# ZrrSkywalker/MonoDETR

Measured on NVIDIA H100. Metric: images/sec (1280x384, fwd+bwd), higher is better.
Workload: dtype f32 (BF16x3: error-compensated bf16 tensor-core products, fp32 accumulate)

## Files before the change

monodetr_b200/csrc/msda.cu:

```cuda
#include <cuda_runtime.h>
#include <stdint.h>

#include "../../include/monodetr_b200.h"
#include "launch.cuh"

namespace {

using namespace mdb;

constexpr int kMaxLevels = 8;
constexpr int kThreads = 256;

struct LevelInfo {
    int H[kMaxLevels];
    int W[kMaxLevels];
    int start[kMaxLevels];
};

__device__ __forceinline__ float4 ldg4(const float* p) { return __ldg(reinterpret_cast<const float4*>(p)); }

__device__ __forceinline__ void red_add_v4(float* addr, float a, float b, float c, float d) {
    asm volatile("red.global.add.v4.f32 [%0], {%1, %2, %3, %4};" ::"l"(addr), "f"(a), "f"(b), "f"(c), "f"(d)
                 : "memory");
}

__device__ __forceinline__ float fma_t(float a, float b, float c) { return fmaf(a, b, c); }
__device__ __forceinline__ double fma_t(double a, double b, double c) { return fma(a, b, c); }
__device__ __forceinline__ float floor_t(float a) { return floorf(a); }
__device__ __forceinline__ double floor_t(double a) { return floor(a); }

template <int LPU>
__global__ void __launch_bounds__(kThreads)
msda_fwd_vec_kernel(const float* __restrict__ value, const int64_t* __restrict__ shapes,
                    const int64_t* __restrict__ lsi, const float* __restrict__ loc,
                    const float* __restrict__ attn, int S, int M, int L, int Lq, long long n_units,
                    long long units_per_block, float* __restrict__ out) {
    constexpr int D = 4 * LPU;
    constexpr int UPW = 32 / LPU;
    constexpr int P = 4;
    __shared__ LevelInfo lv;
    if (threadIdx.x < L) {
        lv.H[threadIdx.x] = (int)shapes[2 * threadIdx.x];
        lv.W[threadIdx.x] = (int)shapes[2 * threadIdx.x + 1];
        lv.start[threadIdx.x] = (int)lsi[threadIdx.x];
    }
    __syncthreads();

    const int lane = threadIdx.x & 31;
    const int sub = lane / LPU;
    const int cl = lane % LPU;
    const int wib = threadIdx.x >> 5;
    const int pix = M * D;
    const long long u_begin = (long long)blockIdx.x * units_per_block;
    const long long u_end = min(n_units, u_begin + units_per_block);
// ... 134 lines not shown
#pragma unroll 1
        for (int half = 0; half < 2; ++half) {
            float2 xy = __ldg(reinterpret_cast<const float2*>(loc + (size_t)u * (L * P * 2)) + half * 8 + cl);
            float a;
            if constexpr (FUSED) {
                a = half ? e1 : e0;
                const int l = half ? lB : lA;
                const float* r = ref + ((size_t)(u / M) * L + l) * ref_dim;
                if (ref_dim == 2) {
                    xy.x = __ldg(r) + xy.x / (float)(half ? WB : WA);
                    xy.y = __ldg(r + 1) + xy.y / (float)(half ? HB : HA);
                } else {
                    xy.x = fmaf(xy.x, (__ldg(r + 2) + __ldg(r + 3)) * 0.5f / (float)P, __ldg(r));
                    xy.y = fmaf(xy.y, (__ldg(r + 4) + __ldg(r + 5)) * 0.5f / (float)P, __ldg(r + 1));
                }
            } else {
                a = __ldg(attn + (size_t)u * (L * P) + half * 8 + cl);
            }
            const PointSetup Sx = half ? setup_point(xy.x, xy.y, a, HB, WB, sB, pix) : setup_point(xy.x, xy.y, a, HA, WA, sA, pix);
#pragma unroll
            for (int jg = 0; jg < 4; ++jg) {
                float4 v[2][4];
                float w[2][4];
#pragma unroll
                for (int jj = 0; jj < 2; ++jj) {
                    const int j = jg * 2 + jj;
                    const int o00 = __shfl_sync(0xffffffffu, Sx.o00, j, 8);
                    const int dxo = __shfl_sync(0xffffffffu, Sx.dxo, j, 8);
                    const int dyo = __shfl_sync(0xffffffffu, Sx.dyo, j, 8);
#pragma unroll
                    for (int k = 0; k < 4; ++k) w[jj][k] = __shfl_sync(0xffffffffu, Sx.w[k], j, 8);
                    const float* p00 = vb + o00;
                    v[jj][0] = ldg4(p00);
                    v[jj][1] = ldg4(p00 + dxo);
                    v[jj][2] = ldg4(p00 + dyo);
                    v[jj][3] = ldg4(p00 + dyo + dxo);
                }
#pragma unroll
                for (int jj = 0; jj < 2; ++jj) {
#pragma unroll
                    for (int k = 0; k < 4; ++k) {
                        acc.x = fmaf(w[jj][k], v[jj][k].x, acc.x);
                        acc.y = fmaf(w[jj][k], v[jj][k].y, acc.y);
                        acc.z = fmaf(w[jj][k], v[jj][k].z, acc.z);
                        acc.w = fmaf(w[jj][k], v[jj][k].w, acc.w);
                    }
                }
            }
        }
        if (live) *reinterpret_cast<float4*>(out + (size_t)unit * D + cl * 4) = acc;
    }
}

template <int LPU, int L, bool FUSED = false, bool REFGRAD = false>
__global__ void __launch_bounds__(kThreads, 2)
msda_bwd_vec_kernel(const float* __restrict__ value, const int64_t* __restrict__ shapes,
                    const int64_t* __restrict__ lsi, const float* __restrict__ loc,
                    const float* __restrict__ attn, const float* __restrict__ grad_out, int S, int M,
                    int Lq, long long n_units, long long units_per_block, float* __restrict__ grad_value,
                    float* __restrict__ grad_loc, float* __restrict__ grad_attn, const float* __restrict__ ref = nullptr,
                    int ref_dim = 0, float* __restrict__ ref_part = nullptr) {
    static_assert(!FUSED || (LPU == 8 && L == 4), "fused pre-processing: D = 32, L = 4");
    static_assert(!REFGRAD || FUSED, "box partials: fused path only");
    constexpr int D = 4 * LPU;
    constexpr int UPW = 32 / LPU;
    constexpr int P = 4;
    constexpr int NLOC = 2 * L * P;
    constexpr int NV = 3 * L * P;
    constexpr int PER = NV / LPU;
    static_assert(NV % LPU == 0 && NLOC % LPU == 0, "butterfly needs divisibility");
    __shared__ LevelInfo lv;
    if (threadIdx.x < L) {
        lv.H[threadIdx.x] = (int)shapes[2 * threadIdx.x];
        lv.W[threadIdx.x] = (int)shapes[2 * threadIdx.x + 1];
        lv.start[threadIdx.x] = (int)lsi[threadIdx.x];
    }
    __syncthreads();

    const int lane = threadIdx.x & 31;
    const int sub = lane / LPU;
    const int cl = lane % LPU;
    const int wib = threadIdx.x >> 5;
    const int pix = M * D;
    const long long u_begin = (long long)blockIdx.x * units_per_block;
    const long long u_end = min(((n_units + UPW - 1) / UPW) * UPW, u_begin + units_per_block);

    for (long long unit = u_begin + wib * UPW + sub; unit < u_end; unit += (kThreads / 32) * UPW) {
        const bool live = unit < n_units;
        const long long u = live ? unit : 0;
        const int m = (int)(u % M);
        const long long b = u / ((long long)Lq * M);
        const size_t vbase = ((size_t)b * S * M + m) * D + cl * 4;
        const float* lp = loc + (size_t)u * L * P * 2;
        const float* ap = attn + (size_t)u * L * P;
        float4 g = ldg4(grad_out + (size_t)u * D + cl * 4);
        if (!live) g = make_float4(0.f, 0.f, 0.f, 0.f);
        [[maybe_unused]] float pa[2] = {0.f, 0.f}, px[2] = {0.f, 0.f}, py[2] = {0.f, 0.f};
        [[maybe_unused]] float sc[L][2];
        if constexpr (FUSED) {
            const float l0 = __ldg(ap + cl), l1 = __ldg(ap + 8 + cl);
            float mx = fmaxf(l0, l1);
            mx = fmaxf(mx, __shfl_xor_sync(0xffffffffu, mx, 4, 8));
            mx = fmaxf(mx, __shfl_xor_sync(0xffffffffu, mx, 2, 8));
            mx = fmaxf(mx, __shfl_xor_sync(0xffffffffu, mx, 1, 8));
            pa[0] = expf(l0 - mx); pa[1] = expf(l1 - mx);
            float sum = pa[0] + pa[1];
            sum += __shfl_xor_sync(0xffffffffu, sum, 4, 8);
            sum += __shfl_xor_sync(0xffffffffu, sum, 2, 8);
            sum += __shfl_xor_sync(0xffffffffu, sum, 1, 8);
            const float inv = 1.f / sum;
            pa[0] *= inv; pa[1] *= inv;
#pragma unroll
            for (int hf = 0; hf < 2; ++hf) {
                const int l = 2 * hf + (cl >> 2);
                const float2 o = __ldg(reinterpret_cast<const float2*>(lp) + hf * 8 + cl);
                const float* r = ref + ((size_t)(u / M) * L + l) * ref_dim;
                if (ref_dim == 2) {
                    px[hf] = __ldg(r) + o.x / (float)lv.W[l];
                    py[hf] = __ldg(r + 1) + o.y / (float)lv.H[l];
                } else {
                    px[hf] = fmaf(o.x, (__ldg(r + 2) + __ldg(r + 3)) * 0.5f / (float)P, __ldg(r));
                    py[hf] = fmaf(o.y, (__ldg(r + 4) + __ldg(r + 5)) * 0.5f / (float)P, __ldg(r + 1));
                }
            }
        }

        float vals[NV];
#pragma unroll
        for (int l = 0; l < L; ++l) {
            const int H = lv.H[l], W = lv.W[l];
            const size_t lbase = vbase + (size_t)lv.start[l] * pix;
            const float4 xy01 = ldg4(lp + l * 8);
            const float4 xy23 = ldg4(lp + l * 8 + 4);
            const float4 a4 = ldg4(ap + l * 4);
            float xs[4] = {xy01.x, xy01.z, xy23.x, xy23.z};
            float ys[4] = {xy01.y, xy01.w, xy23.y, xy23.w};
            float as[4] = {a4.x, a4.y, a4.z, a4.w};
            if constexpr (FUSED) {
                if (ref_dim == 2) {
                    sc[l][0] = 1.f / (float)W; sc[l][1] = 1.f / (float)H;
                } else {
                    const float* r = ref + ((size_t)(u / M) * L + l) * ref_dim;
                    sc[l][0] = (__ldg(r + 2) + __ldg(r + 3)) * 0.5f / (float)P;
                    sc[l][1] = (__ldg(r + 4) + __ldg(r + 5)) * 0.5f / (float)P;
                }
#pragma unroll
                for (int p = 0; p < P; ++p) {
                    xs[p] = __shfl_sync(0xffffffffu, px[l >> 1], 4 * (l & 1) + p, 8);
                    ys[p] = __shfl_sync(0xffffffffu, py[l >> 1], 4 * (l & 1) + p, 8);
                    as[p] = __shfl_sync(0xffffffffu, pa[l >> 1], 4 * (l & 1) + p, 8);
                }
            }
#pragma unroll
            for (int p = 0; p < P; ++p) {
                const float x = fmaf(xs[p], (float)W, -0.5f);
                const float y = fmaf(ys[p], (float)H, -0.5f);
                const bool inside = live && (y > -1.f) && (x > -1.f) && (y < (float)H) && (x < (float)W);
                const float xf = floorf(x), yf = floorf(y);
                const int x0 = (int)xf, y0 = (int)yf;
                const float lx = x - xf, ly = y - yf, hx = 1.f - lx, hy = 1.f - ly;
                const bool top = inside && (y0 >= 0), bot = inside && (y0 + 1 <= H - 1);
                const bool lef = (x0 >= 0), rig = (x0 + 1 <= W - 1);
                const long long o00 = (long long)lbase + ((long long)y0 * W + x0) * pix;
                const long long o01 = o00 + pix, o10 = o00 + (long long)W * pix, o11 = o10 + pix;
                const float4 z = make_float4(0.f, 0.f, 0.f, 0.f);
                const float4 v1 = (top && lef) ? ldg4(value + o00) : z;
                const float4 v2 = (top && rig) ? ldg4(value + o01) : z;
                const float4 v3 = (bot && lef) ? ldg4(value + o10) : z;
                const float4 v4 = (bot && rig) ? ldg4(value + o11) : z;
                const float a = as[p];
                const float w1 = hy * hx, w2 = hy * lx, w3 = ly * hx, w4 = ly * lx;
                const float tx = g.x * a, ty = g.y * a, tz = g.z * a, tw = g.w * a;
                if (top && lef) red_add_v4(grad_value + o00, w1 * tx, w1 * ty, w1 * tz, w1 * tw);
                if (top && rig) red_add_v4(grad_value + o01, w2 * tx, w2 * ty, w2 * tz, w2 * tw);
                if (bot && lef) red_add_v4(grad_value + o10, w3 * tx, w3 * ty, w3 * tz, w3 * tw);
                if (bot && rig) red_add_v4(grad_value + o11, w4 * tx, w4 * ty, w4 * tz, w4 * tw);
                float ga = 0.f, gx = 0.f, gy = 0.f;
#define MDB_ACC(c)                                                                   \
    ga = fmaf(g.c, w1 * v1.c + w2 * v2.c + w3 * v3.c + w4 * v4.c, ga);               \
    gx = fmaf(g.c * a, hy * (v2.c - v1.c) + ly * (v4.c - v3.c), gx);                 \
    gy = fmaf(g.c * a, hx * (v3.c - v1.c) + lx * (v4.c - v2.c), gy);
                MDB_ACC(x) MDB_ACC(y) MDB_ACC(z) MDB_ACC(w)
#undef MDB_ACC
                const int jx = (l * P + p) * 2, jy = jx + 1, ja = NLOC + l * P + p;
                vals[(jx % LPU) * PER + jx / LPU] = gx * (float)W;
                vals[(jy % LPU) * PER + jy / LPU] = gy * (float)H;
                vals[(ja % LPU) * PER + ja / LPU] = ga;
            }
        }
        {
            int n = NV;
#pragma unroll
            for (int off = LPU / 2; off >= 1; off >>= 1) {
                n >>= 1;
                const bool up = (cl & off) != 0;
#pragma unroll
                for (int i = 0; i < NV / 2; ++i) {
                    if (i < n) {
                        const float send = up ? vals[i] : vals[i + n];
                        const float keep = up ? vals[i + n] : vals[i];
                        vals[i] = keep + __shfl_xor_sync(0xffffffffu, send, off);
                    }
                }
            }
        }
        if constexpr (FUSED) {
            const float a0 = pa[0], a1 = pa[1];
            float dot = a0 * vals[4] + a1 * vals[5];
            dot += __shfl_xor_sync(0xffffffffu, dot, 4, 8);
            dot += __shfl_xor_sync(0xffffffffu, dot, 2, 8);
            dot += __shfl_xor_sync(0xffffffffu, dot, 1, 8);
            if (live) {
                float* gl = grad_loc + (size_t)unit * NLOC;
                float* gat = grad_attn + (size_t)unit * (L * P);
#pragma unroll
                for (int i = 0; i < 4; ++i) gl[i * 8 + cl] = vals[i] * ((cl & 1) ? sc[i][1] : sc[i][0]);
                gat[cl] = a0 * (vals[4] - dot);
                gat[8 + cl] = a1 * (vals[5] - dot);
            }
            if constexpr (REFGRAD) {
                float* rp = ref_part + (size_t)unit * (L * 4);
#pragma unroll
                for (int i = 0; i < 4; ++i) {
                    float s = vals[i], w = vals[i] * __ldg(lp + i * 8 + cl);
                    s += __shfl_xor_sync(0xffffffffu, s, 2, 8);
                    w += __shfl_xor_sync(0xffffffffu, w, 2, 8);
                    s += __shfl_xor_sync(0xffffffffu, s, 4, 8);
                    w += __shfl_xor_sync(0xffffffffu, w, 4, 8);
                    if (live && cl < 2) {
                        rp[i * 4 + cl] = s;
                        rp[i * 4 + 2 + cl] = w;
                    }
                }
            }
        } else if (live) {
            float* gl = grad_loc + (size_t)unit * NLOC;
            float* gat = grad_attn + (size_t)unit * (L * P);
#pragma unroll
            for (int i = 0; i < PER; ++i) {
                const int j = i * LPU + cl;
                if (i * LPU < NLOC) gl[j] = vals[i];
                else gat[j - NLOC] = vals[i];
            }
        }
    }
}


template <typename T>
__global__ void __launch_bounds__(kThreads)
msda_fwd_generic_kernel(const T* __restrict__ value, const int64_t* __restrict__ shapes,
                        const int64_t* __restrict__ lsi, const T* __restrict__ loc,
                        const T* __restrict__ attn, int S, int M, int D, int L, int Lq, int P,
                        long long n_units, T* __restrict__ out) {
    const int lane = threadIdx.x & 31;
    const long long warp = (long long)blockIdx.x * (kThreads / 32) + (threadIdx.x >> 5);
    const long long nwarps = (long long)gridDim.x * (kThreads / 32);
    const size_t pix = (size_t)M * D;
    for (long long unit = warp; unit < n_units; unit += nwarps) {
        const int m = (int)(unit % M);
        const long long b = unit / ((long long)Lq * M);
        for (int c0 = 0; c0 < D; c0 += 32) {
            const int c = c0 + lane;
            const bool cok = c < D;
            T acc = 0;
            for (int l = 0; l < L; ++l) {
                const int H = (int)shapes[2 * l], W = (int)shapes[2 * l + 1];
                const T* vl = value + ((size_t)b * S + (size_t)lsi[l]) * pix + (size_t)m * D + (cok ? c : 0);
                for (int p = 0; p < P; ++p) {
                    const size_t pi = ((size_t)unit * L + l) * P + p;
                    const T a = attn[pi];
                    const T x = fma_t(loc[2 * pi], (T)W, (T)-0.5);
                    const T y = fma_t(loc[2 * pi + 1], (T)H, (T)-0.5);
                    if (!(y > (T)-1 && x > (T)-1 && y < (T)H && x < (T)W)) continue;
                    const T xf = floor_t(x), yf = floor_t(y);
                    const int x0 = (int)xf, y0 = (int)yf;
                    const T lx = x - xf, ly = y - yf, hx = (T)1 - lx, hy = (T)1 - ly;
                    const bool top = y0 >= 0, bot = y0 + 1 <= H - 1, lef = x0 >= 0, rig = x0 + 1 <= W - 1;
                    const long long o00 = ((long long)y0 * W + x0) * (long long)pix;
                    T v1 = 0, v2 = 0, v3 = 0, v4 = 0;
                    if (cok) {
                        if (top && lef) v1 = vl[o00];
                        if (top && rig) v2 = vl[o00 + (long long)pix];
                        if (bot && lef) v3 = vl[o00 + (long long)W * pix];
                        if (bot && rig) v4 = vl[o00 + (long long)W * pix + pix];
                    }
                    acc += a * ((hy * hx) * v1 + (hy * lx) * v2 + (ly * hx) * v3 + (ly * lx) * v4);
                }
            }
            if (cok) out[(size_t)unit * D + c] = acc;
        }
    }
}

template <typename T>
__device__ __forceinline__ T warp_sum(T v) {
#pragma unroll
    for (int off = 16; off >= 1; off >>= 1) v += __shfl_xor_sync(0xffffffffu, v, off);
    return v;
}
// ... 50 lines not shown
                    grad_loc[2 * pi + 1] = (T)H * gy;
                }
            }
        }
    }
}

template <typename T>
__global__ void __launch_bounds__(kThreads)
msda_bwd_value_ordered_kernel(const int64_t* __restrict__ shapes, const int64_t* __restrict__ lsi, const T* __restrict__ loc,
                              const T* __restrict__ attn, const T* __restrict__ grad_out, int S, int M, int D, int L, int Lq,
                              int P, T* grad_value) {
    const int l = (int)(blockIdx.x % L);
    const int m = (int)((blockIdx.x / L) % M);
    const long long b = blockIdx.x / ((long long)L * M);
    const int H = (int)shapes[2 * l], W = (int)shapes[2 * l + 1];
    const size_t pix = (size_t)M * D;
    const size_t lbase = ((size_t)b * S + (size_t)lsi[l]) * pix + (size_t)m * D;
    for (int c = threadIdx.x; c < D; c += blockDim.x) {
        for (int q = 0; q < Lq; ++q) {
            const size_t unit = ((size_t)b * Lq + q) * M + m;
            const T g = grad_out[unit * D + c];
            for (int p = 0; p < P; ++p) {
                const size_t pi = (unit * L + l) * P + p;
                const T x = fma_t(loc[2 * pi], (T)W, (T)-0.5);
                const T y = fma_t(loc[2 * pi + 1], (T)H, (T)-0.5);
                if (!(y > (T)-1 && x > (T)-1 && y < (T)H && x < (T)W)) continue;
                const T tg = g * attn[pi];
                const T xf = floor_t(x), yf = floor_t(y);
                const int x0 = (int)xf, y0 = (int)yf;
                const T lx = x - xf, ly = y - yf, hx = (T)1 - lx, hy = (T)1 - ly;
                const bool top = y0 >= 0, bot = y0 + 1 <= H - 1, lef = x0 >= 0, rig = x0 + 1 <= W - 1;
                const long long o00 = (long long)lbase + ((long long)y0 * W + x0) * (long long)pix + c;
                const long long o01 = o00 + (long long)pix, o10 = o00 + (long long)W * pix, o11 = o10 + pix;
                if (top && lef) grad_value[o00] += (hy * hx) * tg;
                if (top && rig) grad_value[o01] += (hy * lx) * tg;
                if (bot && lef) grad_value[o10] += (ly * hx) * tg;
                if (bot && rig) grad_value[o11] += (ly * lx) * tg;
            }
        }
    }
}

int check_common(const void* a, const void* b, const void* c, const void* d, const void* e, int B, int S,
                 int M, int D, int L, int Lq, int P) {
    if (B < 0 || S < 0 || M < 0 || D < 0 || L < 0 || Lq < 0 || P < 0) return MDB_EINVAL;
    const long long n = (long long)B * Lq * M * D;
    if (n > 0 && L > 0 && P > 0 && (!a || !b || !c || !d || !e)) return MDB_EINVAL;
    return 0;
}

bool aligned16(const void* p) { return (reinterpret_cast<uintptr_t>(p) & 15u) == 0; }

template <typename T>
int forward_impl(const T* value, const int64_t* shapes, const int64_t* lsi, const T* loc, const T* attn, int B,
                 int S, int M, int D, int L, int Lq, int P, T* out, void* stream_) {
    int rc = check_common(value, shapes, lsi, loc, attn, B, S, M, D, L, Lq, P);
    if (rc) return rc;
    cudaStream_t stream = static_cast<cudaStream_t>(stream_);
    const long long n_units = (long long)B * Lq * M;
    if (n_units == 0 || D == 0) return 0;
    if (!out) return MDB_EINVAL;
    if (L == 0 || P == 0) {
        return (int)cudaMemsetAsync(out, 0, sizeof(T) * (size_t)n_units * D, stream);
    }
    if constexpr (sizeof(T) == 4) {
        const bool fast = (P == 4) && (L <= kMaxLevels) && (D == 16 || D == 32 || D == 64) && aligned16(value) &&
                          aligned16(loc) && aligned16(attn) && aligned16(out);
        if (fast) {
            const int lpu = D / 4, upw = 32 / lpu;
            const int grid = grid_cap((n_units + upw - 1) / upw, kThreads / 32, num_sms() * 8);
            const long long per = (kThreads / 32) * upw;
            const long long upb = ((n_units + grid - 1) / grid + per - 1) / per * per;
            if (lpu == 8 && L == 4)
                msda_fwd_d32_kernel<false><<<grid, kThreads, 0, stream>>>(value, shapes, lsi, loc, attn, nullptr, 0, S, M, Lq, n_units, upb, out);
            else if (lpu == 8)
                msda_fwd_vec_kernel<8><<<grid, kThreads, 0, stream>>>(value, shapes, lsi, loc, attn, S, M, L, Lq, n_units, upb, out);
            else if (lpu == 4)
                msda_fwd_vec_kernel<4><<<grid, kThreads, 0, stream>>>(value, shapes, lsi, loc, attn, S, M, L, Lq, n_units, upb, out);
            else
                msda_fwd_vec_kernel<16><<<grid, kThreads, 0, stream>>>(value, shapes, lsi, loc, attn, S, M, L, Lq, n_units, upb, out);
            return (int)cudaGetLastError();
        }
    }
    const int grid = grid_cap(n_units, kThreads / 32, num_sms() * 8);
    msda_fwd_generic_kernel<T><<<grid, kThreads, 0, stream>>>(value, shapes, lsi, loc, attn, S, M, D, L, Lq, P, n_units, out);
    return (int)cudaGetLastError();
}

template <typename T>
int backward_impl(const T* value, const int64_t* shapes, const int64_t* lsi, const T* loc, const T* attn,
                  const T* grad_out, int B, int S, int M, int D, int L, int Lq, int P, T* grad_value, T* grad_loc,
                  T* grad_attn, void* stream_) {
    int rc = check_common(value, shapes, lsi, loc, attn, B, S, M, D, L, Lq, P);
    if (rc) return rc;
    cudaStream_t stream = static_cast<cudaStream_t>(stream_);
    const long long n_units = (long long)B * Lq * M;
    const size_t nv = (size_t)B * S * M * D;
    if (nv) {
        if (!grad_value) return MDB_EINVAL;
        cudaError_t e = cudaMemsetAsync(grad_value, 0, sizeof(T) * nv, stream);
        if (e != cudaSuccess) return (int)e;
    }
    if (n_units == 0 || L == 0 || P == 0) return 0;
    if (!grad_loc || !grad_attn) return MDB_EINVAL;
    if (D == 0) {
        cudaError_t e = cudaMemsetAsync(grad_loc, 0, sizeof(T) * (size_t)n_units * L * P * 2, stream);
        if (e != cudaSuccess) return (int)e;
        return (int)cudaMemsetAsync(grad_attn, 0, sizeof(T) * (size_t)n_units * L * P, stream);
    }
    if (!grad_out) return MDB_EINVAL;
    if (mdb_get_deterministic()) {
        const int grid = grid_cap(n_units, kThreads / 32, num_sms() * 8);
        msda_bwd_generic_kernel<T, false><<<grid, kThreads, 0, stream>>>(value, shapes, lsi, loc, attn, grad_out, S, M, D, L, Lq, P, n_units, grad_value, grad_loc, grad_attn);
        cudaError_t e = cudaGetLastError();
        if (e != cudaSuccess) return (int)e;
        int threads = (D + 31) / 32 * 32;
        if (threads > kThreads) threads = kThreads;
        msda_bwd_value_ordered_kernel<T><<<(unsigned)((long long)B * M * L), threads, 0, stream>>>(shapes, lsi, loc, attn, grad_out, S, M, D, L, Lq, P, grad_value);
        return (int)cudaGetLastError();
    }
    if constexpr (sizeof(T) == 4) {
        const bool fast = (P == 4) && (L == 4) && (D == 16 || D == 32 || D == 64) && aligned16(value) &&
                          aligned16(loc) && aligned16(attn) && aligned16(grad_out) && aligned16(grad_value);
        if (fast) {
            const int lpu = D / 4, upw = 32 / lpu;
            const int grid = grid_cap((n_units + upw - 1) / upw, kThreads / 32, num_sms() * 6);
            const long long per = (kThreads / 32) * upw;
            const long long upb = ((n_units + grid - 1) / grid + per - 1) / per * per;
            if (lpu == 8)
                msda_bwd_vec_kernel<8, 4><<<grid, kThreads, 0, stream>>>(value, shapes, lsi, loc, attn, grad_out, S, M, Lq, n_units, upb, grad_value, grad_loc, grad_attn);
            else if (lpu == 4)
                msda_bwd_vec_kernel<4, 4><<<grid, kThreads, 0, stream>>>(value, shapes, lsi, loc, attn, grad_out, S, M, Lq, n_units, upb, grad_value, grad_loc, grad_attn);
            else
                msda_bwd_vec_kernel<16, 4><<<grid, kThreads, 0, stream>>>(value, shapes, lsi, loc, attn, grad_out, S, M, Lq, n_units, upb, grad_value, grad_loc, grad_attn);
            return (int)cudaGetLastError();
        }
    }
    const int grid = grid_cap(n_units, kThreads / 32, num_sms() * 8);
    msda_bwd_generic_kernel<T><<<grid, kThreads, 0, stream>>>(value, shapes, lsi, loc, attn, grad_out, S, M, D, L, Lq, P, n_units, grad_value, grad_loc, grad_attn);
    return (int)cudaGetLastError();
}

}

extern "C" {

int mdb_msda_forward_f32(const float* value, const int64_t* spatial_shapes, const int64_t* level_start,
                         const float* sampling_loc, const float* attn_weight, int B, int S, int M, int D, int L,
                         int Lq, int P, float* out, void* stream) {
    return forward_impl<float>(value, spatial_shapes, level_start, sampling_loc, attn_weight, B, S, M, D, L, Lq, P, out, stream);
}
int mdb_msda_forward_f64(const double* value, const int64_t* spatial_shapes, const int64_t* level_start,
                         const double* sampling_loc, const double* attn_weight, int B, int S, int M, int D, int L,
                         int Lq, int P, double* out, void* stream) {
    return forward_impl<double>(value, spatial_shapes, level_start, sampling_loc, attn_weight, B, S, M, D, L, Lq, P, out, stream);
}
int mdb_msda_backward_f32(const float* value, const int64_t* spatial_shapes, const int64_t* level_start,
                          const float* sampling_loc, const float* attn_weight, const float* grad_out, int B, int S,
                          int M, int D, int L, int Lq, int P, float* grad_value, float* grad_loc, float* grad_attn,
                          void* stream) {
    return backward_impl<float>(value, spatial_shapes, level_start, sampling_loc, attn_weight, grad_out, B, S, M, D, L, Lq, P, grad_value, grad_loc, grad_attn, stream);
}
int mdb_msda_fused_forward_f32(const float* value, const int64_t* spatial_shapes, const int64_t* level_start, const float* offsets,
                               const float* logits, const float* ref, int B, int S, int M, int D, int L, int Lq, int P, int ref_dim,
                               float* out, void* stream_) {
    if (D != 32 || L != 4 || P != 4 || (ref_dim != 2 && ref_dim != 6)) return MDB_EUNSUPPORTED;
    int rc = check_common(value, spatial_shapes, level_start, offsets, logits, B, S, M, D, L, Lq, P);
    if (rc) return rc;
    const long long n_units = (long long)B * Lq * M;
    if (n_units == 0) return 0;
    if (!ref || !out) return MDB_EINVAL;
    if (!aligned16(value) || !aligned16(offsets) || !aligned16(logits) || !aligned16(out)) return MDB_EUNSUPPORTED;
    const int grid = grid_cap((n_units + 3) / 4, kThreads / 32, num_sms() * 8);
    const long long per = (kThreads / 32) * 4;
    const long long upb = ((n_units + grid - 1) / grid + per - 1) / per * per;
    msda_fwd_d32_kernel<true><<<grid, kThreads, 0, static_cast<cudaStream_t>(stream_)>>>(value, spatial_shapes, level_start, offsets, logits, ref,
                                                                                         ref_dim, S, M, Lq, n_units, upb, out);
    return (int)cudaGetLastError();
}
int mdb_msda_fused_backward_f32(const float* value, const int64_t* spatial_shapes, const int64_t* level_start, const float* offsets,
                                const float* logits, const float* ref, const float* grad_out, int B, int S, int M, int D, int L, int Lq,
                                int P, int ref_dim, float* grad_value, float* grad_offsets, float* grad_logits, void* stream_) {
    if (D != 32 || L != 4 || P != 4 || (ref_dim != 2 && ref_dim != 6)) return MDB_EUNSUPPORTED;
    if (mdb_get_deterministic()) return MDB_EUNSUPPORTED;
    int rc = check_common(value, spatial_shapes, level_start, offsets, logits, B, S, M, D, L, Lq, P);
    if (rc) return rc;
    cudaStream_t stream = static_cast<cudaStream_t>(stream_);
    const long long n_units = (long long)B * Lq * M;
    const size_t nv = (size_t)B * S * M * D;
    if (!aligned16(value) || !aligned16(offsets) || !aligned16(logits) || !aligned16(grad_out) || !aligned16(grad_value))
        return MDB_EUNSUPPORTED;
    if (nv) {
        if (!grad_value) return MDB_EINVAL;
        cudaError_t e = cudaMemsetAsync(grad_value, 0, sizeof(float) * nv, stream);
        if (e != cudaSuccess) return (int)e;
    }
    if (n_units == 0) return 0;
    if (!ref || !grad_out || !grad_offsets || !grad_logits) return MDB_EINVAL;
    const int grid = grid_cap((n_units + 3) / 4, kThreads / 32, num_sms() * 6);
    const long long per = (kThreads / 32) * 4;
    const long long upb = ((n_units + grid - 1) / grid + per - 1) / per * per;
    msda_bwd_vec_kernel<8, 4, true><<<grid, kThreads, 0, stream>>>(value, spatial_shapes, level_start, offsets, logits, grad_out, S, M, Lq, n_units,
                                                                   upb, grad_value, grad_offsets, grad_logits, ref, ref_dim);
    return (int)cudaGetLastError();
}
int mdb_msda_fused_backward_ref_f32(const float* value, const int64_t* spatial_shapes, const int64_t* level_start,
                                    const float* offsets, const float* logits, const float* ref, const float* grad_out, int B, int S,
                                    int M, int D, int L, int Lq, int P, int ref_dim, float* grad_value, float* grad_offsets,
                                    float* grad_logits, float* ref_part, void* stream_) {
    if (D != 32 || L != 4 || P != 4 || ref_dim != 6) return MDB_EUNSUPPORTED;
    if (mdb_get_deterministic()) return MDB_EUNSUPPORTED;
    int rc = check_common(value, spatial_shapes, level_start, offsets, logits, B, S, M, D, L, Lq, P);
    if (rc) return rc;
    cudaStream_t stream = static_cast<cudaStream_t>(stream_);
    const long long n_units = (long long)B * Lq * M;
    const size_t nv = (size_t)B * S * M * D;
    if (!aligned16(value) || !aligned16(offsets) || !aligned16(logits) || !aligned16(grad_out) || !aligned16(grad_value))
        return MDB_EUNSUPPORTED;
    if (nv) {
        if (!grad_value) return MDB_EINVAL;
        cudaError_t e = cudaMemsetAsync(grad_value, 0, sizeof(float) * nv, stream);
        if (e != cudaSuccess) return (int)e;
    }
    if (n_units == 0) return 0;
    if (!ref || !grad_out || !grad_offsets || !grad_logits || !ref_part) return MDB_EINVAL;
    const int grid = grid_cap((n_units + 3) / 4, kThreads / 32, num_sms() * 6);
    const long long per = (kThreads / 32) * 4;
    const long long upb = ((n_units + grid - 1) / grid + per - 1) / per * per;
    msda_bwd_vec_kernel<8, 4, true, true><<<grid, kThreads, 0, stream>>>(value, spatial_shapes, level_start, offsets, logits, grad_out, S, M,
                                                                         Lq, n_units, upb, grad_value, grad_offsets, grad_logits, ref,
                                                                         ref_dim, ref_part);
    return (int)cudaGetLastError();
}
int mdb_msda_backward_f64(const double* value, const int64_t* spatial_shapes, const int64_t* level_start,
                          const double* sampling_loc, const double* attn_weight, const double* grad_out, int B, int S,
                          int M, int D, int L, int Lq, int P, double* grad_value, double* grad_loc, double* grad_attn,
                          void* stream) {
    return backward_impl<double>(value, spatial_shapes, level_start, sampling_loc, attn_weight, grad_out, B, S, M, D, L, Lq, P, grad_value, grad_loc, grad_attn, stream);
}

}

namespace {

constexpr int kPrepMaxLP = 16;

__global__ void __launch_bounds__(256)
msda_prep_fwd_kernel(const float* __restrict__ off, const float* __restrict__ logits, const float* __restrict__ ref,
                     const int64_t* __restrict__ shapes, int M, int L, int P, int ref_dim, long long n_units,
                     float* __restrict__ loc, float* __restrict__ attn) {
    const int LP = L * P;
    for (long long u = blockIdx.x * (long long)blockDim.x + threadIdx.x; u < n_units; u += (long long)gridDim.x * blockDim.x) {
        const long long bq = u / M;
        const float* o = off + u * LP * 2;
        const float* lg = logits + u * LP;
        float* lo = loc + u * LP * 2;
        float* at = attn + u * LP;
        float v[kPrepMaxLP];
        float mx = -INFINITY;
        for (int i = 0; i < LP; i += 4) {
            const float4 t = *reinterpret_cast<const float4*>(lg + i);
            v[i] = t.x; v[i + 1] = t.y; v[i + 2] = t.z; v[i + 3] = t.w;
            mx = fmaxf(mx, fmaxf(fmaxf(t.x, t.y), fmaxf(t.z, t.w)));
        }
        float sum = 0.f;
        for (int i = 0; i < LP; ++i) { v[i] = expf(v[i] - mx); sum += v[i]; }
        const float inv = 1.f / sum;
        for (int i = 0; i < LP; i += 4)
            *reinterpret_cast<float4*>(at + i) = make_float4(v[i] * inv, v[i + 1] * inv, v[i + 2] * inv, v[i + 3] * inv);
        for (int l = 0; l < L; ++l) {
            const float* r = ref + (bq * L + l) * ref_dim;
            float sx, sy;
            if (ref_dim == 2) {
                sx = 1.f / (float)shapes[2 * l + 1];
                sy = 1.f / (float)shapes[2 * l];
            } else {
                sx = (r[2] + r[3]) * 0.5f / (float)P;
                sy = (r[4] + r[5]) * 0.5f / (float)P;
            }
            const float rx = r[0], ry = r[1];
            for (int p = 0; p < P; p += 2) {
                const float4 t = *reinterpret_cast<const float4*>(o + (l * P + p) * 2);
                float4 w;
                if (ref_dim == 2) { w.x = rx + t.x / (float)shapes[2 * l + 1]; w.y = ry + t.y / (float)shapes[2 * l];
                                    w.z = rx + t.z / (float)shapes[2 * l + 1]; w.w = ry + t.w / (float)shapes[2 * l]; }
// ... 75 lines not shown
```

Baseline: 173.6.

## Reorder MSDA backward work by batch/head-group slices for L2 locality

Moves the per-unit backward body into a device helper and adds a D=32 kernel whose blocks each own a (batch, group of 4 heads, query chunk) work item. A host planner sizes query chunks so the value and grad_value slices touched concurrently across the grid fit a 24 MiB L2 budget, which keeps atomic reductions and value gathers L2-resident instead of scattering heads across blocks. The trade-off is a fixed grid of 2 blocks per SM, possible load imbalance from chunk rounding, and partially idle lanes when M is not a multiple of 4.

```diff
diff --git a/monodetr_b200/csrc/msda.cu b/monodetr_b200/csrc/msda.cu
--- a/monodetr_b200/csrc/msda.cu
+++ b/monodetr_b200/csrc/msda.cu
@@ -1,5 +1,7 @@
 #include <cuda_runtime.h>
 #include <stdint.h>
+
+#include <algorithm>
 
 #include "../../include/monodetr_b200.h"
 #include "launch.cuh"
@@ -240,23 +242,186 @@
     }
 }
 
-template <int LPU, int L, bool FUSED = false, bool REFGRAD = false>
+template <int LPU, int L, bool FUSED, bool REFGRAD>
+__device__ __forceinline__ void bwd_unit(const LevelInfo& lv, const float* __restrict__ value, const float* __restrict__ loc,
+                                         const float* __restrict__ attn, const float* __restrict__ grad_out, int S, int M, int Lq,
+                                         long long u, bool live, int cl, float* __restrict__ grad_value,
+                                         float* __restrict__ grad_loc, float* __restrict__ grad_attn,
+                                         const float* __restrict__ ref, int ref_dim, float* __restrict__ ref_part) {
+    static_assert(!FUSED || (LPU == 8 && L == 4), "fused pre-processing: D = 32, L = 4");
+    static_assert(!REFGRAD || FUSED, "box partials: fused path only");
+    constexpr int D = 4 * LPU;
+    constexpr int P = 4;
+    constexpr int NLOC = 2 * L * P;
+    constexpr int NV = 3 * L * P;
+    constexpr int PER = NV / LPU;
+    static_assert(NV % LPU == 0 && NLOC % LPU == 0, "butterfly needs divisibility");
+    const int pix = M * D;
+    const int m = (int)(u % M);
+    const long long b = u / ((long long)Lq * M);
+    const size_t vbase = ((size_t)b * S * M + m) * D + cl * 4;
+    const float* lp = loc + (size_t)u * L * P * 2;
+    const float* ap = attn + (size_t)u * L * P;
+    float4 g = ldg4(grad_out + (size_t)u * D + cl * 4);
+    if (!live) g = make_float4(0.f, 0.f, 0.f, 0.f);
+    [[maybe_unused]] float pa[2] = {0.f, 0.f}, px[2] = {0.f, 0.f}, py[2] = {0.f, 0.f};
+    [[maybe_unused]] float sc[L][2];
+    if constexpr (FUSED) {
+        const float l0 = __ldg(ap + cl), l1 = __ldg(ap + 8 + cl);
+        float mx = fmaxf(l0, l1);
+        mx = fmaxf(mx, __shfl_xor_sync(0xffffffffu, mx, 4, 8));
+        mx = fmaxf(mx, __shfl_xor_sync(0xffffffffu, mx, 2, 8));
+        mx = fmaxf(mx, __shfl_xor_sync(0xffffffffu, mx, 1, 8));
+        pa[0] = expf(l0 - mx); pa[1] = expf(l1 - mx);
+        float sum = pa[0] + pa[1];
+        sum += __shfl_xor_sync(0xffffffffu, sum, 4, 8);
+        sum += __shfl_xor_sync(0xffffffffu, sum, 2, 8);
+        sum += __shfl_xor_sync(0xffffffffu, sum, 1, 8);
+        const float inv = 1.f / sum;
+        pa[0] *= inv; pa[1] *= inv;
+#pragma unroll
+        for (int hf = 0; hf < 2; ++hf) {
+            const int l = 2 * hf + (cl >> 2);
+            const float2 o = __ldg(reinterpret_cast<const float2*>(lp) + hf * 8 + cl);
+            const float* r = ref + ((size_t)(u / M) * L + l) * ref_dim;
+            if (ref_dim == 2) {
+                px[hf] = __ldg(r) + o.x / (float)lv.W[l];
+                py[hf] = __ldg(r + 1) + o.y / (float)lv.H[l];
+            } else {
+                px[hf] = fmaf(o.x, (__ldg(r + 2) + __ldg(r + 3)) * 0.5f / (float)P, __ldg(r));
+                py[hf] = fmaf(o.y, (__ldg(r + 4) + __ldg(r + 5)) * 0.5f / (float)P, __ldg(r + 1));
+            }
+        }
+    }
+
+    float vals[NV];
+#pragma unroll
+    for (int l = 0; l < L; ++l) {
+        const int H = lv.H[l], W = lv.W[l];
+        const float4 xy01 = ldg4(lp + l * 8);
+        const float4 xy23 = ldg4(lp + l * 8 + 4);
+        const float4 a4 = ldg4(ap + l * 4);
+        float xs[4] = {xy01.x, xy01.z, xy23.x, xy23.z};
+        float ys[4] = {xy01.y, xy01.w, xy23.y, xy23.w};
+        float as[4] = {a4.x, a4.y, a4.z, a4.w};
+        if constexpr (FUSED) {
+            if (ref_dim == 2) {
+                sc[l][0] = 1.f / (float)W; sc[l][1] = 1.f / (float)H;
+            } else {
+                const float* r = ref + ((size_t)(u / M) * L + l) * ref_dim;
+                sc[l][0] = (__ldg(r + 2) + __ldg(r + 3)) * 0.5f / (float)P;
+                sc[l][1] = (__ldg(r + 4) + __ldg(r + 5)) * 0.5f / (float)P;
+            }
+#pragma unroll
+            for (int p = 0; p < P; ++p) {
+                xs[p] = __shfl_sync(0xffffffffu, px[l >> 1], 4 * (l & 1) + p, 8);
+                ys[p] = __shfl_sync(0xffffffffu, py[l >> 1], 4 * (l & 1) + p, 8);
+                as[p] = __shfl_sync(0xffffffffu, pa[l >> 1], 4 * (l & 1) + p, 8);
+            }
+        }
+#pragma unroll
+        for (int p = 0; p < P; ++p) {
+            const float x = fmaf(xs[p], (float)W, -0.5f);
+            const float y = fmaf(ys[p], (float)H, -0.5f);
+            const bool inside = live && (y > -1.f) && (x > -1.f) && (y < (float)H) && (x < (float)W);
+            const float xf = floorf(x), yf = floorf(y);
+            const int x0 = (int)xf, y0 = (int)yf;
+            const float lx = x - xf, ly = y - yf, hx = 1.f - lx, hy = 1.f - ly;
+            const bool top = inside && (y0 >= 0), bot = inside && (y0 + 1 <= H - 1);
+            const bool lef = (x0 >= 0), rig = (x0 + 1 <= W - 1);
+            const int p00 = lv.start[l] + y0 * W + x0;
+            const long long o00 = (long long)vbase + (long long)p00 * pix;
+            const long long o01 = o00 + pix, o10 = o00 + (long long)W * pix, o11 = o10 + pix;
+            const float4 z = make_float4(0.f, 0.f, 0.f, 0.f);
+            const float4 v1 = (top && lef) ? ldg4(value + o00) : z;
+            const float4 v2 = (top && rig) ? ldg4(value + o01) : z;
+            const float4 v3 = (bot && lef) ? ldg4(value + o10) : z;
+            const float4 v4 = (bot && rig) ? ldg4(value + o11) : z;
+            const float a = as[p];
+            const float w1 = hy * hx, w2 = hy * lx, w3 = ly * hx, w4 = ly * lx;
+            const float4 t = make_float4(g.x * a, g.y * a, g.z * a, g.w * a);
+            if (top && lef) red_add_v4(grad_value + o00, w1 * t.x, w1 * t.y, w1 * t.z, w1 * t.w);
+            if (top && rig) red_add_v4(grad_value + o01, w2 * t.x, w2 * t.y, w2 * t.z, w2 * t.w);
+            if (bot && lef) red_add_v4(grad_value + o10, w3 * t.x, w3 * t.y, w3 * t.z, w3 * t.w);
+            if (bot && rig) red_add_v4(grad_value + o11, w4 * t.x, w4 * t.y, w4 * t.z, w4 * t.w);
+            float ga = 0.f, gx = 0.f, gy = 0.f;
+#define MDB_ACC(c)                                                                   \
+    ga = fmaf(g.c, w1 * v1.c + w2 * v2.c + w3 * v3.c + w4 * v4.c, ga);               \
+    gx = fmaf(g.c * a, hy * (v2.c - v1.c) + ly * (v4.c - v3.c), gx);                 \
+    gy = fmaf(g.c * a, hx * (v3.c - v1.c) + lx * (v4.c - v2.c), gy);
+            MDB_ACC(x) MDB_ACC(y) MDB_ACC(z) MDB_ACC(w)
+#undef MDB_ACC
+            const int jx = (l * P + p) * 2, jy = jx + 1, ja = NLOC + l * P + p;
+            vals[(jx % LPU) * PER + jx / LPU] = gx * (float)W;
+            vals[(jy % LPU) * PER + jy / LPU] = gy * (float)H;
+            vals[(ja % LPU) * PER + ja / LPU] = ga;
+        }
+    }
+    {
+        int n = NV;
+#pragma unroll
+        for (int off = LPU / 2; off >= 1; off >>= 1) {
+            n >>= 1;
+            const bool up = (cl & off) != 0;
+#pragma unroll
+            for (int i = 0; i < NV / 2; ++i) {
+                if (i < n) {
+                    const float send = up ? vals[i] : vals[i + n];
+                    const float keep = up ? vals[i + n] : vals[i];
+                    vals[i] = keep + __shfl_xor_sync(0xffffffffu, send, off);
+                }
+            }
+        }
+    }
+    if constexpr (FUSED) {
+        const float a0 = pa[0], a1 = pa[1];
+        float dot = a0 * vals[4] + a1 * vals[5];
+        dot += __shfl_xor_sync(0xffffffffu, dot, 4, 8);
+        dot += __shfl_xor_sync(0xffffffffu, dot, 2, 8);
+        dot += __shfl_xor_sync(0xffffffffu, dot, 1, 8);
+        if (live) {
+            float* gl = grad_loc + (size_t)u * NLOC;
+            float* gat = grad_attn + (size_t)u * (L * P);
+#pragma unroll
+            for (int i = 0; i < 4; ++i) gl[i * 8 + cl] = vals[i] * ((cl & 1) ? sc[i][1] : sc[i][0]);
+            gat[cl] = a0 * (vals[4] - dot);
+            gat[8 + cl] = a1 * (vals[5] - dot);
+        }
+        if constexpr (REFGRAD) {
+            float* rp = ref_part + (size_t)u * (L * 4);
+#pragma unroll
+            for (int i = 0; i < 4; ++i) {
+                float s = vals[i], w = vals[i] * __ldg(lp + i * 8 + cl);
+                s += __shfl_xor_sync(0xffffffffu, s, 2, 8);
+                w += __shfl_xor_sync(0xffffffffu, w, 2, 8);
+                s += __shfl_xor_sync(0xffffffffu, s, 4, 8);
+                w += __shfl_xor_sync(0xffffffffu, w, 4, 8);
+                if (live && cl < 2) {
+                    rp[i * 4 + cl] = s;
+                    rp[i * 4 + 2 + cl] = w;
+                }
+            }
+        }
+    } else if (live) {
+        float* gl = grad_loc + (size_t)u * NLOC;
+        float* gat = grad_attn + (size_t)u * (L * P);
+#pragma unroll
+        for (int i = 0; i < PER; ++i) {
+            const int j = i * LPU + cl;
+            if (i * LPU < NLOC) gl[j] = vals[i];
+            else gat[j - NLOC] = vals[i];
+        }
+    }
+}
+
+template <int LPU, int L>
 __global__ void __launch_bounds__(kThreads, 2)
 msda_bwd_vec_kernel(const float* __restrict__ value, const int64_t* __restrict__ shapes,
                     const int64_t* __restrict__ lsi, const float* __restrict__ loc,
                     const float* __restrict__ attn, const float* __restrict__ grad_out, int S, int M,
                     int Lq, long long n_units, long long units_per_block, float* __restrict__ grad_value,
-                    float* __restrict__ grad_loc, float* __restrict__ grad_attn, const float* __restrict__ ref = nullptr,
-                    int ref_dim = 0, float* __restrict__ ref_part = nullptr) {
-    static_assert(!FUSED || (LPU == 8 && L == 4), "fused pre-processing: D = 32, L = 4");
-    static_assert(!REFGRAD || FUSED, "box partials: fused path only");
-    constexpr int D = 4 * LPU;
+                    float* __restrict__ grad_loc, float* __restrict__ grad_attn) {
     constexpr int UPW = 32 / LPU;
-    constexpr int P = 4;
-    constexpr int NLOC = 2 * L * P;
-    constexpr int NV = 3 * L * P;
-    constexpr int PER = NV / LPU;
-    static_assert(NV % LPU == 0 && NLOC % LPU == 0, "butterfly needs divisibility");
     __shared__ LevelInfo lv;
     if (threadIdx.x < L) {
         lv.H[threadIdx.x] = (int)shapes[2 * threadIdx.x];
@@ -264,176 +429,51 @@
         lv.start[threadIdx.x] = (int)lsi[threadIdx.x];
     }
     __syncthreads();
-
     const int lane = threadIdx.x & 31;
     const int sub = lane / LPU;
     const int cl = lane % LPU;
     const int wib = threadIdx.x >> 5;
-    const int pix = M * D;
     const long long u_begin = (long long)blockIdx.x * units_per_block;
     const long long u_end = min(((n_units + UPW - 1) / UPW) * UPW, u_begin + units_per_block);
-
     for (long long unit = u_begin + wib * UPW + sub; unit < u_end; unit += (kThreads / 32) * UPW) {
         const bool live = unit < n_units;
-        const long long u = live ? unit : 0;
-        const int m = (int)(u % M);
-        const long long b = u / ((long long)Lq * M);
-        const size_t vbase = ((size_t)b * S * M + m) * D + cl * 4;
-        const float* lp = loc + (size_t)u * L * P * 2;
-        const float* ap = attn + (size_t)u * L * P;
-        float4 g = ldg4(grad_out + (size_t)u * D + cl * 4);
-        if (!live) g = make_float4(0.f, 0.f, 0.f, 0.f);
-        [[maybe_unused]] float pa[2] = {0.f, 0.f}, px[2] = {0.f, 0.f}, py[2] = {0.f, 0.f};
-        [[maybe_unused]] float sc[L][2];
-        if constexpr (FUSED) {
-            const float l0 = __ldg(ap + cl), l1 = __ldg(ap + 8 + cl);
-            float mx = fmaxf(l0, l1);
-            mx = fmaxf(mx, __shfl_xor_sync(0xffffffffu, mx, 4, 8));
-            mx = fmaxf(mx, __shfl_xor_sync(0xffffffffu, mx, 2, 8));
-            mx = fmaxf(mx, __shfl_xor_sync(0xffffffffu, mx, 1, 8));
-            pa[0] = expf(l0 - mx); pa[1] = expf(l1 - mx);
-            float sum = pa[0] + pa[1];
-            sum += __shfl_xor_sync(0xffffffffu, sum, 4, 8);
-            sum += __shfl_xor_sync(0xffffffffu, sum, 2, 8);
-            sum += __shfl_xor_sync(0xffffffffu, sum, 1, 8);
-            const float inv = 1.f / sum;
-            pa[0] *= inv; pa[1] *= inv;
-#pragma unroll
-            for (int hf = 0; hf < 2; ++hf) {
-                const int l = 2 * hf + (cl >> 2);
-                const float2 o = __ldg(reinterpret_cast<const float2*>(lp) + hf * 8 + cl);
-                const float* r = ref + ((size_t)(u / M) * L + l) * ref_dim;
-                if (ref_dim == 2) {
-                    px[hf] = __ldg(r) + o.x / (float)lv.W[l];
-                    py[hf] = __ldg(r + 1) + o.y / (float)lv.H[l];
-                } else {
-                    px[hf] = fmaf(o.x, (__ldg(r + 2) + __ldg(r + 3)) * 0.5f / (float)P, __ldg(r));
-                    py[hf] = fmaf(o.y, (__ldg(r + 4) + __ldg(r + 5)) * 0.5f / (float)P, __ldg(r + 1));
-                }
-            }
-        }
-
-        float vals[NV];
-#pragma unroll
-        for (int l = 0; l < L; ++l) {
-            const int H = lv.H[l], W = lv.W[l];
-            const size_t lbase = vbase + (size_t)lv.start[l] * pix;
-            const float4 xy01 = ldg4(lp + l * 8);
-            const float4 xy23 = ldg4(lp + l * 8 + 4);
-            const float4 a4 = ldg4(ap + l * 4);
-            float xs[4] = {xy01.x, xy01.z, xy23.x, xy23.z};
-            float ys[4] = {xy01.y, xy01.w, xy23.y, xy23.w};
-            float as[4] = {a4.x, a4.y, a4.z, a4.w};
-            if constexpr (FUSED) {
-                if (ref_dim == 2) {
-                    sc[l][0] = 1.f / (float)W; sc[l][1] = 1.f / (float)H;
-                } else {
-                    const float* r = ref + ((size_t)(u / M) * L + l) * ref_dim;
-                    sc[l][0] = (__ldg(r + 2) + __ldg(r + 3)) * 0.5f / (float)P;
-                    sc[l][1] = (__ldg(r + 4) + __ldg(r + 5)) * 0.5f / (float)P;
-                }
-#pragma unroll
-                for (int p = 0; p < P; ++p) {
-                    xs[p] = __shfl_sync(0xffffffffu, px[l >> 1], 4 * (l & 1) + p, 8);
-                    ys[p] = __shfl_sync(0xffffffffu, py[l >> 1], 4 * (l & 1) + p, 8);
-                    as[p] = __shfl_sync(0xffffffffu, pa[l >> 1], 4 * (l & 1) + p, 8);
-                }
-            }
-#pragma unroll
-            for (int p = 0; p < P; ++p) {
-                const float x = fmaf(xs[p], (float)W, -0.5f);
-                const float y = fmaf(ys[p], (float)H, -0.5f);
-                const bool inside = live && (y > -1.f) && (x > -1.f) && (y < (float)H) && (x < (float)W);
-                const float xf = floorf(x), yf = floorf(y);
-                const int x0 = (int)xf, y0 = (int)yf;
-                const float lx = x - xf, ly = y - yf, hx = 1.f - lx, hy = 1.f - ly;
-                const bool top = inside && (y0 >= 0), bot = inside && (y0 + 1 <= H - 1);
-                const bool lef = (x0 >= 0), rig = (x0 + 1 <= W - 1);
-                const long long o00 = (long long)lbase + ((long long)y0 * W + x0) * pix;
-                const long long o01 = o00 + pix, o10 = o00 + (long long)W * pix, o11 = o10 + pix;
-                const float4 z = make_float4(0.f, 0.f, 0.f, 0.f);
-                const float4 v1 = (top && lef) ? ldg4(value + o00) : z;
-                const float4 v2 = (top && rig) ? ldg4(value + o01) : z;
-                const float4 v3 = (bot && lef) ? ldg4(value + o10) : z;
-                const float4 v4 = (bot && rig) ? ldg4(value + o11) : z;
-                const float a = as[p];
-                const float w1 = hy * hx, w2 = hy * lx, w3 = ly * hx, w4 = ly * lx;
-                const float tx = g.x * a, ty = g.y * a, tz = g.z * a, tw = g.w * a;
-                if (top && lef) red_add_v4(grad_value + o00, w1 * tx, w1 * ty, w1 * tz, w1 * tw);
-                if (top && rig) red_add_v4(grad_value + o01, w2 * tx, w2 * ty, w2 * tz, w2 * tw);
-                if (bot && lef) red_add_v4(grad_value + o10, w3 * tx, w3 * ty, w3 * tz, w3 * tw);
-                if (bot && rig) red_add_v4(grad_value + o11, w4 * tx, w4 * ty, w4 * tz, w4 * tw);
-                float ga = 0.f, gx = 0.f, gy = 0.f;
-#define MDB_ACC(c)                                                                   \
-    ga = fmaf(g.c, w1 * v1.c + w2 * v2.c + w3 * v3.c + w4 * v4.c, ga);               \
-    gx = fmaf(g.c * a, hy * (v2.c - v1.c) + ly * (v4.c - v3.c), gx);                 \
-    gy = fmaf(g.c * a, hx * (v3.c - v1.c) + lx * (v4.c - v2.c), gy);
-                MDB_ACC(x) MDB_ACC(y) MDB_ACC(z) MDB_ACC(w)
-#undef MDB_ACC
-                const int jx = (l * P + p) * 2, jy = jx + 1, ja = NLOC + l * P + p;
-                vals[(jx % LPU) * PER + jx / LPU] = gx * (float)W;
-                vals[(jy % LPU) * PER + jy / LPU] = gy * (float)H;
-                vals[(ja % LPU) * PER + ja / LPU] = ga;
-            }
-        }
-        {
-            int n = NV;
-#pragma unroll
-            for (int off = LPU / 2; off >= 1; off >>= 1) {
-                n >>= 1;
-                const bool up = (cl & off) != 0;
-#pragma unroll
-                for (int i = 0; i < NV / 2; ++i) {
-                    if (i < n) {
-                        const float send = up ? vals[i] : vals[i + n];
-                        const float keep = up ? vals[i + n] : vals[i];
-                        vals[i] = keep + __shfl_xor_sync(0xffffffffu, send, off);
-                    }
-                }
-            }
-        }
-        if constexpr (FUSED) {
-            const float a0 = pa[0], a1 = pa[1];
-            float dot = a0 * vals[4] + a1 * vals[5];
-            dot += __shfl_xor_sync(0xffffffffu, dot, 4, 8);
-            dot += __shfl_xor_sync(0xffffffffu, dot, 2, 8);
-            dot += __shfl_xor_sync(0xffffffffu, dot, 1, 8);
-            if (live) {
-                float* gl = grad_loc + (size_t)unit * NLOC;
-                float* gat = grad_attn + (size_t)unit * (L * P);
-#pragma unroll
-                for (int i = 0; i < 4; ++i) gl[i * 8 + cl] = vals[i] * ((cl & 1) ? sc[i][1] : sc[i][0]);
-                gat[cl] = a0 * (vals[4] - dot);
-                gat[8 + cl] = a1 * (vals[5] - dot);
-            }
-            if constexpr (REFGRAD) {
-                float* rp = ref_part + (size_t)unit * (L * 4);
-#pragma unroll
-                for (int i = 0; i < 4; ++i) {
-                    float s = vals[i], w = vals[i] * __ldg(lp + i * 8 + cl);
-                    s += __shfl_xor_sync(0xffffffffu, s, 2, 8);
-                    w += __shfl_xor_sync(0xffffffffu, w, 2, 8);
-                    s += __shfl_xor_sync(0xffffffffu, s, 4, 8);
-                    w += __shfl_xor_sync(0xffffffffu, w, 4, 8);
-                    if (live && cl < 2) {
-                        rp[i * 4 + cl] = s;
-                        rp[i * 4 + 2 + cl] = w;
-                    }
-                }
-            }
-        } else if (live) {
-            float* gl = grad_loc + (size_t)unit * NLOC;
-            float* gat = grad_attn + (size_t)unit * (L * P);
-#pragma unroll
-            for (int i = 0; i < PER; ++i) {
-                const int j = i * LPU + cl;
-                if (i * LPU < NLOC) gl[j] = vals[i];
-                else gat[j - NLOC] = vals[i];
-            }
-        }
-    }
-}
-
+        bwd_unit<LPU, L, false, false>(lv, value, loc, attn, grad_out, S, M, Lq, live ? unit : 0, live, cl, grad_value, grad_loc,
+                                       grad_attn, nullptr, 0, nullptr);
+    }
+}
+
+template <bool FUSED, bool REFGRAD>
+__global__ void __launch_bounds__(kThreads, 2)
+msda_bwd_d32_kernel(const float* __restrict__ value, const int64_t* __restrict__ shapes, const int64_t* __restrict__ lsi,
+                    const float* __restrict__ loc, const float* __restrict__ attn, const float* __restrict__ grad_out, int S,
+                    int M, int Lq, long long n_items, int n_chunks, int chunk, int n_groups, float* __restrict__ grad_value,
+                    float* __restrict__ grad_loc, float* __restrict__ grad_attn, const float* __restrict__ ref = nullptr,
+                    int ref_dim = 0, float* __restrict__ ref_part = nullptr) {
+    constexpr int L = 4;
+    __shared__ LevelInfo lv;
+    if (threadIdx.x < L) {
+        lv.H[threadIdx.x] = (int)shapes[2 * threadIdx.x];
+        lv.W[threadIdx.x] = (int)shapes[2 * threadIdx.x + 1];
+        lv.start[threadIdx.x] = (int)lsi[threadIdx.x];
+    }
+    __syncthreads();
+    const int lane = threadIdx.x & 31;
+    const int sub = lane >> 3, cl = lane & 7;
+    const int wib = threadIdx.x >> 5;
+    for (long long item = blockIdx.x; item < n_items; item += gridDim.x) {
+        const long long bg = item / n_chunks;
+        const int m0 = (int)(bg % n_groups) * 4;
+        const long long b = bg / n_groups;
+        const int q0 = (int)(item % n_chunks) * chunk;
+        const int q1 = min(Lq, q0 + chunk);
+        for (int q = q0 + wib; q < q1; q += kThreads / 32) {
+            const bool live = m0 + sub < M;
+            const long long unit = (b * Lq + q) * M + (live ? m0 + sub : m0);
+            bwd_unit<8, L, FUSED, REFGRAD>(lv, value, loc, attn, grad_out, S, M, Lq, unit, live, cl, grad_value, grad_loc, grad_attn,
+                                           ref, ref_dim, ref_part);
+        }
+    }
+}
 
 template <typename T>
 __global__ void __launch_bounds__(kThreads)
@@ -590,6 +630,46 @@
 
 bool aligned16(const void* p) { return (reinterpret_cast<uintptr_t>(p) & 15u) == 0; }
 
+constexpr long long kL2SliceBudget = 24ll << 20;
+
+struct BwdD32Plan {
+    int grid, n_chunks, chunk, n_groups;
+    long long n_items;
+};
+
+BwdD32Plan plan_bwd_d32(int B, int S, int M, int Lq) {
+    BwdD32Plan pl{};
+    pl.n_groups = (M + 3) / 4;
+    const long long n_bm = (long long)B * pl.n_groups, G = 2ll * num_sms();
+    const long long slice = std::max(1ll, 2ll * S * std::min(M, 4) * 32 * 4);
+    const long long slices = std::max(1ll, kL2SliceBudget / slice);
+    const long long nmin = std::min<long long>(Lq, (G + slices - 1) / slices);
+    long long best = -1;
+    for (long long n = nmin; n <= std::min<long long>(2 * nmin, Lq); ++n) {
+        const long long c = (Lq + n - 1) / n, nn = (Lq + c - 1) / c;
+        const long long cost = ((n_bm * nn + G - 1) / G) * ((c + 7) / 8);
+        if (best < 0 || cost < best) {
+            best = cost;
+            pl.chunk = (int)c;
+            pl.n_chunks = (int)nn;
+        }
+    }
+    pl.n_items = n_bm * pl.n_chunks;
+    pl.grid = (int)std::min(G, pl.n_items);
+    return pl;
+}
+
+template <bool FUSED, bool REFGRAD>
+int launch_bwd_d32(const float* value, const int64_t* shapes, const int64_t* lsi, const float* loc, const float* attn,
+                   const float* grad_out, int B, int S, int M, int Lq, float* grad_value, float* grad_loc, float* grad_attn,
+                   const float* ref, int ref_dim, float* ref_part, cudaStream_t stream) {
+    const BwdD32Plan pl = plan_bwd_d32(B, S, M, Lq);
+    msda_bwd_d32_kernel<FUSED, REFGRAD><<<pl.grid, kThreads, 0, stream>>>(value, shapes, lsi, loc, attn, grad_out, S, M, Lq,
+                                                                         pl.n_items, pl.n_chunks, pl.chunk, pl.n_groups, grad_value, grad_loc,
+                                                                         grad_attn, ref, ref_dim, ref_part);
+    return (int)cudaGetLastError();
+}
+
 template <typename T>
 int forward_impl(const T* value, const int64_t* shapes, const int64_t* lsi, const T* loc, const T* attn, int B,
                  int S, int M, int D, int L, int Lq, int P, T* out, void* stream_) {
@@ -667,8 +747,9 @@
             const long long per = (kThreads / 32) * upw;
             const long long upb = ((n_units + grid - 1) / grid + per - 1) / per * per;
             if (lpu == 8)
-                msda_bwd_vec_kernel<8, 4><<<grid, kThreads, 0, stream>>>(value, shapes, lsi, loc, attn, grad_out, S, M, Lq, n_units, upb, grad_value, grad_loc, grad_attn);
-            else if (lpu == 4)
+                return launch_bwd_d32<false, false>(value, shapes, lsi, loc, attn, grad_out, B, S, M, Lq, grad_value, grad_loc, grad_attn,
+                                                    nullptr, 0, nullptr, stream);
+            if (lpu == 4)
                 msda_bwd_vec_kernel<4, 4><<<grid, kThreads, 0, stream>>>(value, shapes, lsi, loc, attn, grad_out, S, M, Lq, n_units, upb, grad_value, grad_loc, grad_attn);
             else
                 msda_bwd_vec_kernel<16, 4><<<grid, kThreads, 0, stream>>>(value, shapes, lsi, loc, attn, grad_out, S, M, Lq, n_units, upb, grad_value, grad_loc, grad_attn);
@@ -736,12 +817,8 @@
     }
     if (n_units == 0) return 0;
     if (!ref || !grad_out || !grad_offsets || !grad_logits) return MDB_EINVAL;
-    const int grid = grid_cap((n_units + 3) / 4, kThreads / 32, num_sms() * 6);
-    const long long per = (kThreads / 32) * 4;
-    const long long upb = ((n_units + grid - 1) / grid + per - 1) / per * per;
-    msda_bwd_vec_kernel<8, 4, true><<<grid, kThreads, 0, stream>>>(value, spatial_shapes, level_start, offsets, logits, grad_out, S, M, Lq, n_units,
-                                                                   upb, grad_value, grad_offsets, grad_logits, ref, ref_dim);
-    return (int)cudaGetLastError();
+    return launch_bwd_d32<true, false>(value, spatial_shapes, level_start, offsets, logits, grad_out, B, S, M, Lq, grad_value,
+                                       grad_offsets, grad_logits, ref, ref_dim, nullptr, stream);
 }
 int mdb_msda_fused_backward_ref_f32(const float* value, const int64_t* spatial_shapes, const int64_t* level_start,
                                     const float* offsets, const float* logits, const float* ref, const float* grad_out, int B, int S,
@@ -763,13 +840,8 @@
     }
     if (n_units == 0) return 0;
     if (!ref || !grad_out || !grad_offsets || !grad_logits || !ref_part) return MDB_EINVAL;
-    const int grid = grid_cap((n_units + 3) / 4, kThreads / 32, num_sms() * 6);
-    const long long per = (kThreads / 32) * 4;
-    const long long upb = ((n_units + grid - 1) / grid + per - 1) / per * per;
-    msda_bwd_vec_kernel<8, 4, true, true><<<grid, kThreads, 0, stream>>>(value, spatial_shapes, level_start, offsets, logits, grad_out, S, M,
-                                                                         Lq, n_units, upb, grad_value, grad_offsets, grad_logits, ref,
-                                                                         ref_dim, ref_part);
-    return (int)cudaGetLastError();
+    return launch_bwd_d32<true, true>(value, spatial_shapes, level_start, offsets, logits, grad_out, B, S, M, Lq, grad_value,
+                                      grad_offsets, grad_logits, ref, ref_dim, ref_part, stream);
 }
 int mdb_msda_backward_f64(const double* value, const int64_t* spatial_shapes, const int64_t* level_start,
                           const double* sampling_loc, const double* attn_weight, const double* grad_out, int B, int S,
```

Result: no change. 174.4, median of 6 (+0.5%).
